# ivclab/CPG

Measured on AMD Instinct MI355X. Metric: images/sec per CPG train-prune-retrain cycle, VGG16 task-1, higher is better.
Workload: dtype f32; 1 GPU; configs[1]: VGG16-BN custom_vgg 224x224, task-1 CPG cycle (finetune -> prune 0.0->0.1 -> recovery, validate after every 20th train step), batch 256 per GPU; task=1, arch=vgg16, global_batch=256, per_gpu_batch=256, parallelism=dp1, epoch_steps=20

## Files before the change

### cpg_amd/_lib.py

```python
import ctypes
import os
import sys

import torch

_HERE = os.path.dirname(os.path.abspath(__file__))
LIB_PATH = os.environ.get('CPG_HIP_LIB') or os.path.join(_HERE, 'lib', 'libcpg_hip.so')

ABI_VERSION = 3
CPG_OK = 0
CPG_E_KRANGE = 2
CPG_E_INVALID = -1
MODE_FINETUNE = 0
MODE_PRUNE = 1



class ConvDesc(ctypes.Structure):
    _fields_ = [(n, ctypes.c_int32) for n in
                ('N', 'C', 'H', 'W', 'K', 'R', 'S', 'stride_h', 'stride_w', 'pad_h', 'pad_w', 'dil_h', 'dil_w', 'groups')]


class PruneResult(ctypes.Structure):
    _fields_ = [('n_candidates', ctypes.c_int64), ('k', ctypes.c_int64), ('n_released', ctypes.c_int64),
# ... 71 lines not shown
    'cpg_bn_workspace_bytes': (_sz, [_i32, _i32, _i32]),
    'cpg_bn_relu_fwd_train': (_int, [_vp, _vp, _vp, _f32, _f32, _vp, _vp, _vp, _vp, _vp, _i32, _i32, _i32, _i32, _vp, _sz, _vp]),
    'cpg_bn_relu_fwd_eval': (_int, [_vp, _vp, _vp, _vp, _vp, _vp, _i32, _i32, _i32, _i32, _vp]),
    'cpg_bn_relu_pool_fwd': (_int, [_vp, _vp, _vp, _f32, _f32, _vp, _vp, _vp, _vp, _vp, _i32, _i32, _i32, _i32, _i32, _vp, _sz, _vp]),
    'cpg_bn_relu_pool_bwd': (_int, [_vp, _vp, _vp, _vp, _vp, _vp, _vp, _vp, _vp, _i32, _i32, _i32, _i32, _i32, _vp, _sz, _vp]),
    'cpg_bn_relu_bwd': (_int, [_vp, _vp, _vp, _vp, _vp, _vp, _vp, _vp, _vp, _i32, _i32, _i32, _i32, _i32, _vp, _sz, _vp]),
    'cpg_conv2d_winograd': (_i32, [_desc, _i32]),
    'cpg_conv2d_bnstats_tiles': (_i32, [_desc]),
    'cpg_conv2d_fwd_bnstats': (_int, [_desc, _vp, _vp, _vp, _f32, _vp, _vp, _vp, _sz, _vp, _sz, _vp]),
    'cpg_conv2d_fwd_bn_eval_supported': (_i32, [_desc]),
    'cpg_conv2d_fwd_bn_eval': (_int, [_desc, _vp, _vp, _vp, _f32, _vp, _vp, _vp, _vp, _vp, _f32, _i32, _vp, _vp, _vp, _sz, _vp]),
    'cpg_conv2d_bf16_supported': (_i32, [_desc]),
    'cpg_conv2d_bf16_workspace_bytes': (_sz, [_desc]),
    'cpg_conv2d_fwd_bf16': (_int, [_desc, _vp, _vp, _vp, _f32, _vp, _vp, _vp, _sz, _vp]),
    'cpg_conv2d_wgrad_bf16_supported': (_i32, [_desc]),
    'cpg_conv2d_wgrad_bf16_workspace_bytes': (_sz, [_desc]),
    'cpg_conv2d_wgrad_bf16': (_int, [_desc, _vp, _vp, _vp, _vp, _f32, _vp, _vp, _vp, _sz, _vp]),
    'cpg_conv2d_fwd_bf16x3': (_int, [_desc, _vp, _vp, _vp, _f32, _vp, _vp, _vp, _sz, _vp]),
    'cpg_conv2d_dgrad_bf16x3': (_int, [_desc, _vp, _vp, _vp, _f32, _vp, _vp, _sz, _vp]),
    'cpg_conv2d_wgrad_bf16x3': (_int, [_desc, _vp, _vp, _vp, _vp, _f32, _vp, _vp, _vp, _sz, _vp]),
    'cpg_conv2d_dgrad_bf16': (_int, [_desc, _vp, _vp, _vp, _f32, _vp, _vp, _sz, _vp]),
    'cpg_conv2d_dgrad_bnbwd_tiles': (_i32, [_desc]),
    'cpg_conv2d_dgrad_bnbwd': (_int, [_desc, _vp, _vp, _vp, _f32, _vp, _vp, _vp, _vp, _vp, _vp, _vp, _sz, _vp, _sz, _vp]),
    'cpg_bn_bwd_from_partials': (_int, [_vp, _i32, _vp, _vp, _vp, _vp, _vp, _vp, _vp, _vp, _vp, _i32, _i32, _i32, _vp, _sz, _vp]),
    'cpg_bn_bwd_finalize_partials': (_int, [_vp, _i32, _i32, _i32, _i32, _vp, _vp, _vp, _vp]),
    'cpg_stem_bn_supported': (_i32, [_desc]),
    'cpg_stem_bn_tiles': (_i32, [_desc]),
    'cpg_stem_bn_stats': (_int, [_desc, _vp, _vp, _vp, _f32, _vp, _vp, _sz, _vp]),
    'cpg_stem_bn_relu_fwd': (_int, [_desc, _vp, _vp, _vp, _f32, _vp, _vp, _vp, _vp, _vp, _vp, _vp]),
    'cpg_stem_bn_relu_bwd_reduce': (_int, [_desc, _vp, _vp, _vp, _f32, _vp, _vp, _vp, _vp, _vp, _vp, _vp, _sz, _vp]),
    'cpg_stem_bn_relu_bwd_apply': (_int, [_desc, _vp, _vp, _vp, _f32, _vp, _vp, _vp, _vp, _vp, _vp, _vp, _vp, _vp]),
    'cpg_stem_bn_wgrad_workspace': (_sz, [_desc]),
    'cpg_stem_bn_relu_bwd_wgrad': (_int, [_desc, _vp, _vp, _vp, _f32, _vp, _vp, _vp, _vp, _vp, _vp, _vp, _vp, _vp, _vp, _sz, _vp]),
    'cpg_bn_stats_finalize_count': (_int, [_vp, _i32, _i32, _i32, _i32, _f32, _f32, _vp, _vp, _vp, _vp, _vp, _vp]),
    'cpg_bn_stats_finalize': (_int, [_vp, _i32, _i32, _i32, _i32, _f32, _f32, _vp, _vp, _vp, _vp, _vp]),
    'cpg_bn_add_relu_mask_bytes': (_sz, [_i32, _i32, _i32]),
    'cpg_bn_add_relu_fwd': (_int, [_vp, _vp, _vp, _vp, _f32, _f32, _vp, _vp, _vp, _vp, _vp, _i32, _i32, _i32, _i32, _vp, _sz, _vp, _vp]),
    'cpg_bn_relu_pool3_supported': (_i32, [_i32, _i32]),
    'cpg_bn_relu_pool3_fwd': (_int, [_vp] * 6 + [_i32] * 4 + [_vp]),
    'cpg_bn_relu_pool3_bwd': (_int, [_vp] * 9 + [_i32] * 5 + [_vp, _sz, _vp]),
    'cpg_bn_add_relu_bwd': (_int, [_vp] * 11 + [_i32] * 4 + [_vp, _sz, _vp, _vp]),
    'cpg_prelu_fwd': (_int, [_vp, _vp, _vp, _vp, _i32, _i32, _i32, _i32, _vp]),
    'cpg_prelu_bwd_bias': (_int, [_vp] * 6 + [_i32] * 4 + [_vp, _sz, _vp]),
    'cpg_prelu_workspace_bytes': (_sz, [_i32, _i32, _i32]),
    'cpg_prelu_bwd': (_int, [_vp, _vp, _vp, _vp, _vp, _i32, _i32, _i32, _i32, _vp, _sz, _vp]),
    'cpg_image_resample_workspace_bytes': (_sz, [ctypes.POINTER(ResampleItem), _i32]),
    'cpg_image_resample': (_int, [_vp, _i64, ctypes.POINTER(ResampleItem), _i32, _vp, _i64, _vp, _sz, _vp]),
    'cpg_image_to_tensor': (_int, [_vp, _i64, ctypes.POINTER(TensorItem), _i32, _i32, _i32, ctypes.POINTER(_f32), ctypes.POINTER(_f32), _vp,
                                           _i64, _vp]),
    'cpg_pair_distance': (_int, [_vp, _i64, _vp, _i64, _i64, _i32, _i32, _vp, _vp, _vp]),
    'cpg_pair_sweep': (_int, [_vp, _vp, _i64, ctypes.POINTER(_f64), _i32, _i32, _vp, _vp, _vp]),
}
EXPORTS = tuple(_SIGNATURES)

_lib = None


class CpgHipError(RuntimeError):
    def __init__(self, fn, code, text):
        super().__init__('%s failed with status %d: %s' % (fn, code, text))
        self.code = code


def lib():
    global _lib
    if _lib is None:
# ... 103 lines not shown
```

### cpg_amd/csrc/conv3x3_stem.hip

```cpp
#include <algorithm>
#include <type_traits>
#include "cpg_dispatch.h"

using namespace cpg;

namespace {

typedef float f32x2 __attribute__((ext_vector_type(2)));
constexpr int ST_R = 8, ST_W = 32;
constexpr int ST_PW = 36;
constexpr int ST_ROWS = ST_R + 2;
constexpr int ST_CMAX = 3, ST_KS = 14;
constexpr int ST_PATCH = ST_CMAX * ST_ROWS * ST_PW;

struct StemGeom {
    int N, C, K, H, W;
    int tiles_x, tiles_y;
    unsigned ntiles;
};

enum { ST_PLAIN = 0, ST_STATS = 1, ST_STATS_ONLY = 2, ST_BN_RELU = 3, ST_BWD_REDUCE = 4, ST_BWD_APPLY = 5, ST_BWD_WGRAD = 6 };
constexpr int ST_TS = 36;
struct StemBn {
    const float *gamma, *beta, *mean, *invstd;
    const float *coef;
    const float *gz;
};

template <int MODE, int NB = 2, bool RAG = false>
__global__ __launch_bounds__(256, 2)
void k_stem_fwd(StemGeom g, const float *__restrict__ x, const float *__restrict__ w, const float *__restrict__ pm, float thr,
                const float *__restrict__ bias, float *__restrict__ y, float *__restrict__ stats, StemBn bn) {
    constexpr bool STATS = MODE == ST_STATS || MODE == ST_STATS_ONLY || MODE == ST_BWD_REDUCE;
    constexpr bool BN = MODE >= ST_BN_RELU;
    constexpr bool STORE = MODE == ST_PLAIN || MODE == ST_STATS || MODE == ST_BN_RELU || MODE == ST_BWD_APPLY;
    constexpr bool WG = MODE == ST_BWD_WGRAD;
    constexpr bool TWO_PASS = STATS || BN;
    __shared__ float smem_all[4 * ST_PATCH];
    __shared__ __attribute__((aligned(16))) float cst[(MODE >= ST_BWD_REDUCE) ? NB * 32 * 8 : 4];
    const int tid = threadIdx.x, lane = tid & 63, wave = __builtin_amdgcn_readfirstlane(tid >> 6);
    if constexpr (MODE >= ST_BWD_REDUCE) {
        if (tid < NB * 32) {
            const bool kv = tid < g.K;
            cst[tid * 8 + 0] = kv ? bn.mean[tid] : 0.0f, cst[tid * 8 + 1] = kv ? bn.invstd[tid] : 0.0f;
            cst[tid * 8 + 2] = kv ? bn.gamma[tid] : 0.0f, cst[tid * 8 + 3] = kv ? bn.beta[tid] : 0.0f;
            cst[tid * 8 + 4] = (MODE >= ST_BWD_APPLY && kv) ? bn.coef[2 * tid] : 0.0f;
            cst[tid * 8 + 5] = (MODE >= ST_BWD_APPLY && kv) ? bn.coef[2 * tid + 1] : 0.0f;
        }
        __syncthreads();
    }
    const int li = lane & 31, lh = lane >> 5;
    float *smem = smem_all + wave * ST_PATCH;
    const int HW = g.H * g.W, CK = g.C * 9;
    __shared__ __attribute__((aligned(16))) float tsm_all[WG ? 4 * 32 * ST_TS : 4];
    float *tsm = tsm_all + (WG ? wave * 32 * ST_TS : 0);
    const int wk = li < CK ? li : 0, wboff = ((wk / 9) * ST_ROWS + (wk % 9) / 3) * ST_PW + wk % 3 + lh;
    f32x16 accw[WG ? NB : 1];
    if constexpr (WG) {
#pragma unroll
        for (int mb = 0; mb < NB; ++mb)
#pragma unroll
            for (int e = 0; e < 16; ++e) accw[mb][e] = 0.0f;
    }

    constexpr bool ALDS = NB == 3 && TWO_PASS;
    __shared__ float a_lds[ALDS ? NB * ST_KS * 64 : 1];
    float A[ALDS ? 1 : NB][ST_KS];
    int boff[ST_KS];
#pragma unroll
    for (int t = 0; t < ST_KS; ++t) {
        const int k = 2 * t + lh;
        const bool kv = k < CK;
#pragma unroll
        for (int mb = 0; mb < NB; ++mb) {
            const int co = mb * 32 + li;
            float v = 0.0f;
            if (kv && co < g.K) {
                v = w[co * CK + k];
                if (pm != nullptr) v *= binarize(pm[co * CK + k], thr);
            }
            if constexpr (ALDS) {
                if (wave == 0) a_lds[(mb * ST_KS + t) * 64 + lane] = v;
            } else {
                A[mb][t] = v;
            }
        }
        const int kk = kv ? k : 0;
        const int c = kk / 9, r = (kk % 9) / 3, s = kk % 3;
        boff[t] = (c * ST_ROWS + r) * ST_PW + s + li;
    }
    constexpr bool HASB = !BN;
    constexpr bool BPASS = HASB && TWO_PASS && NB == 3;
    float bv[HASB ? (BPASS ? 1 : NB) : 1][HASB ? 16 : 1];
    if constexpr (HASB && !BPASS) {
#pragma unroll
        for (int mb = 0; mb < NB; ++mb)
#pragma unroll
            for (int e = 0; e < 16; ++e) {
                const int co = mb * 32 + (e & 3) + 8 * (e >> 2) + 4 * lh;
                bv[mb][e] = (bias != nullptr && co < g.K) ? bias[co] : 0.0f;
            }
    }

    const __amdgpu_buffer_rsrc_t srd_x = __builtin_amdgcn_make_buffer_rsrc((void *)x, 0, g.N * g.C * HW * 4, 0x00020000);
    constexpr int kOOR = (int)0x80000000;
    const int hw_half = lane >> 5, hcol = lane & 31;
    float pc[15], ph;
    auto tile_coords = [&](unsigned tile, int &n, int &y0, int &x0) {
        const unsigned per_img = (unsigned)(g.tiles_x * g.tiles_y);
        n = (int)(tile / per_img);
        const unsigned r = tile % per_img;
        y0 = (int)(r / (unsigned)g.tiles_x) * ST_R, x0 = (int)(r % (unsigned)g.tiles_x) * ST_W;
    };
    auto issue_loads = [&](unsigned tile) {
        int n, y0, x0;
        tile_coords(tile, n, y0, x0);
#pragma unroll
        for (int q = 0; q < 15; ++q) {
            const int item = 2 * q + hw_half, c = item / ST_ROWS, r = item % ST_ROWS;
            const int row = y0 - 1 + r, col = x0 + hcol;
            const bool ok = c < g.C && (unsigned)row < (unsigned)g.H && col < g.W;
            const int off = ok ? (((n * g.C + c) * g.H + row) * g.W + col) * 4 : kOOR;
            pc[q] = __builtin_bit_cast(float, __builtin_amdgcn_raw_buffer_load_b32(srd_x, off, 0, 0));
        }
        {
            const int item = lane >> 1, side = lane & 1, c = item / ST_ROWS, r = item % ST_ROWS;
            const int row = y0 - 1 + r, col = side ? x0 + ST_W : x0 - 1;
            const bool ok = item < ST_CMAX * ST_ROWS && c < g.C && (unsigned)row < (unsigned)g.H && (unsigned)col < (unsigned)g.W;
            const int off = ok ? (((n * g.C + c) * g.H + row) * g.W + col) * 4 : kOOR;
            ph = __builtin_bit_cast(float, __builtin_amdgcn_raw_buffer_load_b32(srd_x, off, 0, 0));
        }
    };
    auto write_patch = [&]() {
#pragma unroll
        for (int q = 0; q < 15; ++q) smem[(2 * q + hw_half) * ST_PW + 1 + hcol] = pc[q];
        if (lane < 2 * ST_CMAX * ST_ROWS) smem[(lane >> 1) * ST_PW + ((lane & 1) ? ST_W + 1 : 0)] = ph;
    };

    if constexpr (ALDS) __syncthreads();
    const unsigned nwaves = gridDim.x * 4, wid = blockIdx.x * 4 + wave;
    if (wid >= g.ntiles) return;
    const int HW4 = HW * 4;
    issue_loads(wid);
    for (unsigned tile = wid; tile < g.ntiles; tile += nwaves) {
        int n, y0, x0;
        tile_coords(tile, n, y0, x0);
        write_patch();
        if (tile + nwaves < g.ntiles) issue_loads(tile + nwaves);
        float s1[16], s2[16];
        auto zero_sums = [&]() {
            if (STATS) {
#pragma unroll
                for (int e = 0; e < 16; ++e) s1[e] = s2[e] = 0.0f;
// ... 67 lines not shown
            for (int mb = MB0; mb < MB1; ++mb)
#pragma unroll
                for (int e = 0; e < 16; ++e) acc[mb][e] = 0.0f;
            const float *prow = smem + j * ST_PW;
#pragma unroll
            for (int t = 0; t < ST_KS; ++t) {
                const float b = prow[boff[t]];
#pragma unroll
                for (int mb = MB0; mb < MB1; ++mb) acc[mb] = __builtin_amdgcn_mfma_f32_32x32x2f32(A[ALDS ? 0 : mb][t], b, acc[mb], 0, 0, 0);
            }
#pragma unroll
            for (int mb = MB0; mb < MB1; ++mb)
#pragma unroll
                for (int e = 0; e < 16; ++e) {
                    const int cu = mb * 32 + (e & 3) + 8 * (e >> 2);
                    const float v = HASB ? acc[mb][e] + bv[(HASB && !BPASS) ? mb : 0][HASB ? e : 0] : acc[mb][e];
                    if constexpr (MODE == ST_PLAIN || MODE == ST_STATS) {
                        __builtin_amdgcn_raw_buffer_store_b32(__builtin_bit_cast(int, v), srd_y, voff_of(mb, e), cu * HW4, 0);
                    }
                    if constexpr (MODE == ST_STATS || MODE == ST_STATS_ONLY) {
                        const float vm = (FULL || pok) ? v : 0.0f;
                        s1[e] += vm;
                        s2[e] = fmaf(vm, vm, s2[e]);
                    }
                    if constexpr (MODE == ST_BN_RELU) {
                        const float z = fmaxf((v - cm[e]) * cis[e] * cga[e] + cbe[e], 0.0f);
                        __builtin_amdgcn_raw_buffer_store_b32(__builtin_bit_cast(int, z), srd_y, voff_of(mb, e), cu * HW4, 0);
                    }
                    if constexpr (MODE >= ST_BWD_REDUCE) {
                        const float *cc = cst + (cu + 4 * lh) * 8 + copq;
                        const f32x4 c4 = *reinterpret_cast<const f32x4 *>(cc);
                        const float xh = (v - c4[0]) * c4[1];
                        const float gm = ((v - c4[0]) * c4[1] * c4[2] + c4[3] > 0.0f) ? gzv[e] : 0.0f;
                        if constexpr (MODE == ST_BWD_REDUCE) {
                            s1[e] += gm;
                            s2[e] = fmaf(gm, xh, s2[e]);
                        } else {
                            const f32x2 c2 = *reinterpret_cast<const f32x2 *>(cc + 4);
                            float gyv = (gm - c2[0] - xh * c2[1]) * (c4[1] * c4[2]);
                            if constexpr (MODE == ST_BWD_APPLY) {
                                __builtin_amdgcn_raw_buffer_store_b32(__builtin_bit_cast(int, gyv), srd_y, voff_of(mb, e), cu * HW4, 0);
                            } else {
                                if (!FULL && !pok) gyv = 0.0f;
                                tsm[((e & 3) + 8 * (e >> 2) + 4 * lh) * ST_TS + (li & 1) * 16 + (li >> 1)] = gyv;
                            }
                        }
                    }
                }
            if constexpr (WG) {
                f32x4 ga[4];
#pragma unroll
                for (int q = 0; q < 4; ++q) ga[q] = *reinterpret_cast<const f32x4 *>(tsm + li * ST_TS + lh * 16 + 4 * q);
                const float *brow = smem + j * ST_PW + wboff;
#pragma unroll
                for (int t = 0; t < 16; ++t)
                    accw[MB0] = __builtin_amdgcn_mfma_f32_32x32x2f32(ga[t >> 2][t & 3], brow[2 * t], accw[MB0], 0, 0, 0);
            }
        };
        auto rows = [&](auto mbsel) {
            if (full) {
#pragma unroll 1
                for (int j = 0; j < ST_R; ++j) row(j, std::true_type{}, mbsel);
            } else {
#pragma unroll 1
                for (int j = 0; j < ST_R; ++j) row(j, std::false_type{}, mbsel);
            }
        };
        auto stats_out = [&](int mb) {
#pragma unroll
            for (int e = 0; e < 16; e += 8) half_wave_sum8(s1 + e), half_wave_sum8(s2 + e);
            if (li == kHalfSumLane) {
#pragma unroll
                for (int e = 0; e < 16; ++e) {
                    const int co = mb * 32 + (e & 3) + 8 * (e >> 2) + 4 * lh;
                    if (RAG && co >= g.K) continue;
                    f32x2 o;
                    o[0] = s1[e], o[1] = s2[e];
                    *reinterpret_cast<f32x2 *>(stats + ((int64_t)co * g.ntiles + tile) * 2) = o;
                }
            }
        };
        if (TWO_PASS) {
            load_bn(0);
            zero_sums();
            rows(std::integral_constant<int, 0>{});
            if (STATS) stats_out(0);
            load_bn(1);
            zero_sums();
            rows(std::integral_constant<int, 1>{});
            if (STATS) stats_out(1);
            if constexpr (NB == 3) {
                load_bn(2);
                zero_sums();
                rows(std::integral_constant<int, 2>{});
                if (STATS) stats_out(2);
            }
        } else {
            rows(std::integral_constant<int, -1>{});
        }
    }
    if constexpr (WG) {
        float *dstw = y + (int64_t)wid * g.K * CK;
#pragma unroll
        for (int mb = 0; mb < NB; ++mb)
#pragma unroll
            for (int e = 0; e < 16; ++e) {
                const int co = mb * 32 + (e & 3) + 8 * (e >> 2) + 4 * lh;
                if (li < CK && co < g.K) dstw[co * CK + li] = accw[mb][e];
            }
    }
}

#define STEM_LAUNCH(MODE, grid, block, shm, stream, ...)                                                          \
    do {                                                                                                          \
        if (g.K == 64) hipLaunchKernelGGL((k_stem_fwd<MODE, 2, false>), grid, block, shm, stream, __VA_ARGS__);   \
        else hipLaunchKernelGGL((k_stem_fwd<MODE, 3, true>), grid, block, shm, stream, __VA_ARGS__);              \
    } while (0)

bool stem_geom(int N, int C, int K, int H, int W, StemGeom &g) {
    if (opt_on(OPT_NO_STEM)) return false;
    if (N < 1 || C < 1 || C > ST_CMAX || K < 64 || K > 96 || H < 1 || W < 1) return false;
    if ((int64_t)N * C * H * W * 4 >= (1ll << 31) || (int64_t)K * H * W * 4 >= (1ll << 31)) return false;
    g.N = N, g.C = C, g.K = K, g.H = H, g.W = W;
    g.tiles_x = (W + ST_W - 1) / ST_W, g.tiles_y = (H + ST_R - 1) / ST_R;
    const int64_t nt = (int64_t)N * g.tiles_x * g.tiles_y;
    if (nt >= (1ll << 31)) return false;
    g.ntiles = (unsigned)nt;
    return true;
}

}

extern "C" int cpg_conv3x3_stem_ok(int N, int C, int K, int H, int W) {
    StemGeom g;
    return stem_geom(N, C, K, H, W, g) ? 1 : 0;
}

extern "C" int cpg_conv3x3_stem_tiles(int N, int C, int K, int H, int W) {
    StemGeom g;
    return stem_geom(N, C, K, H, W, g) ? (int)g.ntiles : 0;
}

// ... 78 lines not shown
    if (!stem_bn_geom(d, g)) return fail(CPG_E_UNSUPPORTED, "cpg_stem_bn_relu_bwd_apply: shape not supported");
    if (bias != nullptr) return fail(CPG_E_UNSUPPORTED, "cpg_stem_bn_relu_bwd_apply: the fused stem takes no conv bias");
    STEM_LAUNCH(ST_BWD_APPLY, dim3(stem_blocks(g)), dim3(256), 0, (hipStream_t)stream_v, g, x, w, pm, thr, bias, gy,
                       (float *)nullptr, StemBn{gamma, beta, mean, invstd, coef, gz});
    CPG_CHECK_LAUNCH("cpg_stem_bn_relu_bwd_apply");
    return CPG_OK;
}

extern "C" size_t cpg_stem_bn_wgrad_workspace(const cpg_conv_desc *d) {
    StemGeom g;
    if (d == nullptr || !stem_bn_geom(d, g)) return 0;
    return (size_t)stem_blocks(g) * 4 * g.K * g.C * 9 * sizeof(float);
}
extern "C" int cpg_stem_bn_relu_bwd_wgrad(const cpg_conv_desc *d, const float *x, const float *w, const float *pm, float thr,
                                          const float *bias, const float *gamma, const float *beta, const float *mean, const float *invstd,
                                          const float *coef, const float *gz, float *gw, float *gpm, void *ws, size_t ws_bytes,
                                          void *stream_v) {
    StemGeom g;
    CPG_REQUIRE(d && x && w && gamma && beta && mean && invstd && coef && gz && gw && ws, "cpg_stem_bn_relu_bwd_wgrad: null pointer");
    CPG_REQUIRE((pm == nullptr) == (gpm == nullptr), "cpg_stem_bn_relu_bwd_wgrad: piggymask and its gradient come as a pair");
    if (!stem_bn_geom(d, g)) return fail(CPG_E_UNSUPPORTED, "cpg_stem_bn_relu_bwd_wgrad: shape not supported");
    if (bias != nullptr) return fail(CPG_E_UNSUPPORTED, "cpg_stem_bn_relu_bwd_wgrad: the fused stem takes no conv bias");
    const unsigned blocks = stem_blocks(g);
    if (ws_bytes < (size_t)blocks * 4 * g.K * g.C * 9 * sizeof(float)) return fail(CPG_E_WORKSPACE, "cpg_stem_bn_relu_bwd_wgrad: workspace too small");
    hipStream_t stream = (hipStream_t)stream_v;
    STEM_LAUNCH(ST_BWD_WGRAD, dim3(blocks), dim3(256), 0, stream, g, x, w, pm, thr, bias, (float *)ws, (float *)nullptr,
                       StemBn{gamma, beta, mean, invstd, coef, gz});
    const int nsplit = (int)std::min<int64_t>((int64_t)g.ntiles, (int64_t)blocks * 4);
    Epilogue ep{gw, nullptr, BIAS_NONE, 1, 1, pm, w, gpm, thr};
    launch_split_reduce((const float *)ws, nsplit, (int64_t)g.K * g.C * 9, 0, ep, stream);
    CPG_CHECK_LAUNCH("cpg_stem_bn_relu_bwd_wgrad");
    return CPG_OK;
}
```

### cpg_amd/csrc/cpg_common.cpp

```cpp
#include "cpg_common.h"
#include <stdarg.h>
#include <stdlib.h>
#include <string.h>
#include <atomic>

namespace cpg {

static thread_local char g_err[512] = "";

char *err_buf() { return g_err; }

int fail(int code, const char *fmt, ...) {
    va_list ap;
    va_start(ap, fmt);
    vsnprintf(g_err, sizeof(g_err), fmt, ap);
    va_end(ap);
    return code;
}

static thread_local PackCtx g_pack = {};
PackCtx &pack_ctx() { return g_pack; }
static thread_local WgradRider g_rider = {};
WgradRider &wgrad_rider() { return g_rider; }

// ... 2 lines not shown
    if (c.mode == PACK_QUERY) {
        c.job = job;
        c.hit = true;
        return 1;
    }
    if (c.mode == PACK_USE && !c.hit) {
        if (c.use == nullptr || c.use_bytes != job.bytes || (((uintptr_t)c.use) & 15) != 0)
            return fail(CPG_E_INVALID, "%s: the packed operand handed in (%zu bytes) is not the one this launch streams (%zu bytes, 16-byte aligned)",
                        what, c.use_bytes, job.bytes);
        *pre = c.use;
        c.hit = true;
        return 2;
    }
    return 0;
}

static std::atomic<int> g_shared_chip{0};
int shared_chip_hint() { return g_shared_chip.load(std::memory_order_relaxed); }

namespace {
enum Kind { BOOL, INT, WINO_KERNEL };
struct OptDef {
    const char *name;
    Kind kind;
};
const OptDef kDefs[OPT_COUNT] = {
    {"CPG_NO_WINO", BOOL},          {"CPG_NO_WINO_WGRAD", BOOL},   {"CPG_NO_WINO_ODD", BOOL},      {"CPG_NO_STEM", BOOL},
    {"CPG_NO_STEM_FUSE", BOOL},     {"CPG_NO_DEAD_SKIP", BOOL},    {"CPG_NO_S2", BOOL},            {"CPG_NO_V14", BOOL},
    {"CPG_DISABLE_CONV3X3", BOOL},  {"CPG_DISABLE_CONV1X1", BOOL}, {"CPG_DISABLE_CONV1X1_WGRAD", BOOL}, {"CPG_DISABLE_PW_GEMM", BOOL},
    {"CPG_C3_FORCE", INT},          {"CPG_C3W_BPC", INT},          {"CPG_W3_PICK", INT},           {"CPG_PWW_BPC", INT},
    {"CPG_STEM_BLOCKS", INT},       {"CPG_WINO_KERNEL", WINO_KERNEL}, {"CPG_WINO_NW", INT},        {"CPG_WINO_PERSIST", INT},
    {"CPG_WINO_GRIDS", INT},        {"CPG_WW_UNITS", INT},         {"CPG_WW_XCD", INT},            {"CPG_PW_TILE", INT},           {"CPG_WG3_SHARE", INT},
    {"CPG_WW_SHARE", INT},          {"CPG_WINO_TAIL", INT},         {"CPG_FC_SMALL", INT},
    {"CPG_NO_WW_RIDER", BOOL},
};

struct Table {
    std::atomic<int> v[OPT_COUNT];
    Table() {
        for (int i = 0; i < OPT_COUNT; ++i) {
            int val = OPT_UNSET;
            if (const char *f = getenv(kDefs[i].name)) {
                switch (kDefs[i].kind) {
                    case BOOL: val = (f[0] == 0 || (f[0] == '0' && f[1] == 0)) ? 0 : 1; break;
                    case INT: val = atoi(f); break;
                    case WINO_KERNEL: val = f[0] == 'b' ? 0 : f[0] == 'p' ? 2 : f[0] == '6' ? 3 : 1; break;
                }
            }
            v[i].store(val, std::memory_order_relaxed);
        }
    }
};
Table g_opts;

int find_opt(const char *name) {
    if (name == nullptr) return -1;
    for (int i = 0; i < OPT_COUNT; ++i)
        if (strcmp(name, kDefs[i].name) == 0) return i;
    return -1;
}
}

int opt(Opt o) { return g_opts.v[o].load(std::memory_order_relaxed); }

}

extern "C" int cpg_set_shared_chip_hint(int32_t shared) {
// ... 19 lines not shown
```

### cpg_amd/csrc/cpg_common.h

```cpp
#pragma once
#include <hip/hip_runtime.h>
#include <stdint.h>
#include <stdio.h>
#include "../../include/cpg_hip.h"

namespace cpg {

char *err_buf();
int fail(int code, const char *fmt, ...);
int shared_chip_hint();

enum Opt {
    OPT_NO_WINO,
    OPT_NO_WINO_WGRAD,
    OPT_NO_WINO_ODD,
    OPT_NO_STEM,
    OPT_NO_STEM_FUSE,
    OPT_NO_DEAD_SKIP,
    OPT_NO_S2,
    OPT_NO_V14,
    OPT_DISABLE_CONV3X3,
    OPT_DISABLE_CONV1X1,
    OPT_DISABLE_CONV1X1_WGRAD,
    OPT_DISABLE_PW_GEMM,
    OPT_C3_FORCE,
    OPT_C3W_BPC,
    OPT_W3_PICK,
    OPT_PWW_BPC,
    OPT_STEM_BLOCKS,
    OPT_WINO_KERNEL,
    OPT_WINO_NW,
    OPT_WINO_PERSIST,
    OPT_WINO_GRIDS,
    OPT_WW_UNITS,
    OPT_WW_XCD,
    OPT_PW_TILE,
    OPT_WG3_SHARE,
    OPT_WW_SHARE,
    OPT_WINO_TAIL,
    OPT_FC_SMALL,
    OPT_NO_WW_RIDER,
    OPT_COUNT
};
constexpr int OPT_UNSET = INT32_MIN;
int opt(Opt o);
inline bool opt_on(Opt o) { const int v = opt(o); return v != OPT_UNSET && v != 0; }
inline int opt_or(Opt o, int dflt) { const int v = opt(o); return v == OPT_UNSET ? dflt : v; }

struct PackJob {
    int family;
    int K, C;
    int a, b, c, d;
    long long total;
    size_t bytes;
};
enum { PACK_NONE = 0, PACK_QUERY = 1, PACK_USE = 2 };
struct PackCtx {
    int mode;
    bool hit;
    PackJob job;
    const float *use;
    size_t use_bytes;
};
PackCtx &pack_ctx();
inline bool pack_query() { return pack_ctx().mode == PACK_QUERY; }
int pack_site(const PackJob &job, const float **pre, const char *what);
int pack_jobs_launch(const PackJob *ja, float *dst_a, const PackJob *jb, float *dst_b, const float *w, const float *pm, float thr,
                     hipStream_t stream);

struct WgradRider {
    bool armed;
    const float *y, *gz, *table;
    float *gy;
    int N, C, HW;
// ... 47 lines not shown
```

### cpg_amd/models/fused_bn.py

```python
import ctypes

import torch
import torch.nn as nn

from .. import _lib
from .layers import BiasGradSink, BnBwdHint, _conv_desc

ENABLED = True
ENABLE_BWD_HINT = False
ENABLE_WGRAD_RIDER = True
RELU_BYTE_MASK = True
FUSE_STEM = True
FUSE_STEM_WGRAD = True
FUSE_SKIP_ADD = True


def _batch_stats(stats, nbt, N, C, HW, eps, momentum, running_mean, running_var, training, device):
    if not training:
        return running_mean, torch.rsqrt(running_var + eps), nbt
    mean = torch.empty(C, dtype=torch.float32, device=device)
    invstd = torch.empty(C, dtype=torch.float32, device=device)
    if stats is not None:
        args = (_lib.dptr(stats, name='bn partial sums'), stats.shape[1], N, C, HW, float(eps), float(momentum),
                _lib.dptr(running_mean, name='running_mean'), _lib.dptr(running_var, name='running_var'), _lib.dptr(mean), _lib.dptr(invstd))
# ... 338 lines not shown
    @staticmethod
    def forward(ctx, x, weight, pm, thr, gamma, beta, running_mean, running_var, eps, momentum, nbt=None):
        x = x.contiguous()
        w = weight.contiguous()
        p = None if pm is None else pm.contiguous()
        d = _conv_desc(x.shape, w.shape, (1, 1), (1, 1), (1, 1), 1)
        s = _lib.stream_ptr()
        thr = float(thr)
        N, K, H, W = x.shape[0], w.shape[0], x.shape[2], x.shape[3]
        tiles = _lib.lib().cpg_stem_bn_tiles(ctypes.byref(d))
        stats = torch.empty((K, tiles, 2), dtype=torch.float32, device=x.device)
        _lib.call('cpg_stem_bn_stats', ctypes.byref(d), _lib.dptr(x, name='input'), _lib.dptr(w, name='weight'), _lib.dptr(p, name='piggymask'),
                  thr, None, _lib.dptr(stats), stats.numel() * 4, s)
        mean, invstd, nbt = _batch_stats(stats, nbt, N, K, H * W, eps, momentum, running_mean, running_var, True, x.device)
        z = torch.empty((N, K, H, W), dtype=torch.float32, device=x.device)
        _lib.call('cpg_stem_bn_relu_fwd', ctypes.byref(d), _lib.dptr(x), _lib.dptr(w), _lib.dptr(p), thr, None, _lib.dptr(gamma, name='bn.weight'),
                  _lib.dptr(beta, name='bn.bias'), _lib.dptr(mean), _lib.dptr(invstd), _lib.dptr(z), s)
        _count(nbt)
        ctx.save_for_backward(x, w, p, gamma, beta, mean, invstd)
        ctx.desc, ctx.thr, ctx.tiles = d, thr, tiles
        return z

    @staticmethod
    def backward(ctx, gz):
        x, w, p, gamma, beta, mean, invstd = ctx.saved_tensors
        d, thr, tiles = ctx.desc, ctx.thr, ctx.tiles
        gz = gz.contiguous()
        L = _lib.lib()
        s = _lib.stream_ptr()
        N, K, H, W = x.shape[0], w.shape[0], x.shape[2], x.shape[3]
        partials = torch.empty((K, tiles, 2), dtype=torch.float32, device=x.device)
        args = (ctypes.byref(d), _lib.dptr(x), _lib.dptr(w), _lib.dptr(p), thr, None, _lib.dptr(gamma), _lib.dptr(beta), _lib.dptr(mean),
                _lib.dptr(invstd))
        _lib.call('cpg_stem_bn_relu_bwd_reduce', *args, _lib.dptr(gz, name='grad_output'), _lib.dptr(partials), partials.numel() * 4, s)
        dgamma, dbeta = torch.empty_like(gamma), torch.empty_like(beta)
        coef = torch.empty(2 * K, dtype=torch.float32, device=x.device)
        _lib.call('cpg_bn_bwd_finalize_partials', _lib.dptr(partials), tiles, N, K, H * W, _lib.dptr(dgamma), _lib.dptr(dbeta), _lib.dptr(coef), s)
        gw = gpm = None
        if ctx.needs_input_grad[1] or (p is not None and ctx.needs_input_grad[2]):
            gw = torch.empty_like(w)
            gpm = None if p is None else torch.empty_like(p)
            if FUSE_STEM_WGRAD:
                ws, nbytes = _lib.workspace(L.cpg_stem_bn_wgrad_workspace(ctypes.byref(d)), x.device)
                _lib.call('cpg_stem_bn_relu_bwd_wgrad', *args, _lib.dptr(coef), _lib.dptr(gz), _lib.dptr(gw), _lib.dptr(gpm), _lib.dptr(ws),
                          nbytes, s)
            else:
                gy = torch.empty((N, K, H, W), dtype=torch.float32, device=x.device)
                _lib.call('cpg_stem_bn_relu_bwd_apply', *args, _lib.dptr(coef), _lib.dptr(gz), _lib.dptr(gy), s)
                ws, nbytes = _lib.workspace(L.cpg_conv2d_workspace_bytes(ctypes.byref(d)), x.device)
                _lib.call('cpg_conv2d_wgrad', ctypes.byref(d), _lib.dptr(x), _lib.dptr(gy), _lib.dptr(w), _lib.dptr(p), thr, _lib.dptr(gw),
                          _lib.dptr(gpm), None, _lib.dptr(ws), nbytes, s)
        return (None, gw, gpm, None, dgamma, dbeta) + (None,) * 5


def stem_conv_bn_relu(conv, bn, x):
    if not (ENABLED and FUSE_STEM and FusedSequential.fuse and hasattr(conv, 'forward_with_bn_stats')
            and _stats_from_conv(bn, FusedSequential.fuse_stats, x, need_grad=True)
            and x.dim() == 4 and x.dtype == torch.float32 and not x.requires_grad
            and conv.bias is None and conv._math() == 'fp32' and tuple(conv.kernel_size) == (3, 3) and tuple(conv.stride) == (1, 1)
            and tuple(conv.padding) == (1, 1) and tuple(conv.dilation) == (1, 1) and conv.groups == 1 and x.shape[0] > 0
            and x.shape[1] == conv.weight.shape[1] and bn.weight.dtype == torch.float32):
        return None
    d = _conv_desc(x.shape, conv.weight.shape, (1, 1), (1, 1), (1, 1), 1)
    if not _lib.lib().cpg_stem_bn_supported(ctypes.byref(d)):
        return None
    return _StemConvBnReluFn.apply(x, conv.weight, conv.piggymask, conv.info['threshold'], bn.weight, bn.bias, bn.running_mean, bn.running_var,
                                   bn.eps, bn.momentum, bn.num_batches_tracked)


def conv_bn_act_skip(conv, bn, act, x):
    if (ENABLED and FUSE_SKIP_ADD and hasattr(conv, 'forward_with_skip') and x.is_cuda and torch.is_grad_enabled() and x.requires_grad
            and conv._math() == 'fp32' and conv.kernel_size == (1, 1) and conv.stride == (1, 1) and conv.in_channels % 16 == 0
            and conv.out_channels % 16 == 0):
        y, stats, skip = conv.forward_with_skip(x)
        if (stats is not None and _stats_from_conv(bn, FusedSequential.fuse_stats) and (act is None or type(act) is nn.ReLU)
# ... 83 lines not shown
```

### include/cpg_hip.h

```cpp
#ifndef CPG_HIP_H
#define CPG_HIP_H

#include <stddef.h>
#include <stdint.h>

#ifdef __cplusplus
extern "C" {
#endif

#define CPG_ABI_VERSION 3

#define CPG_OK 0
#define CPG_E_INVALID (-1)
#define CPG_E_UNSUPPORTED (-2)
#define CPG_E_WORKSPACE (-3)
#define CPG_E_KRANGE 2
#define CPG_E_HIP_BASE 1000

#define CPG_MODE_FINETUNE 0
#define CPG_MODE_PRUNE 1

typedef struct cpg_conv_desc {
    int32_t N, C, H, W;
    int32_t K;
// ... 145 lines not shown
                        const float *bias, float *y, void *workspace, size_t workspace_bytes, void *stream);
int cpg_conv2d_dgrad_bf16(const cpg_conv_desc *desc, const float *gy, const float *w, const float *piggymask, float threshold,
                          float *gx, void *workspace, size_t workspace_bytes, void *stream);

int32_t cpg_conv2d_dgrad_bnbwd_tiles(const cpg_conv_desc *desc);
int cpg_conv2d_dgrad_bnbwd(const cpg_conv_desc *desc, const float *gy, const float *w, const float *piggymask, float threshold,
                           const float *ypre, const float *gamma, const float *beta, const float *mean, const float *invstd,
                           float *gm, float *partials, size_t partial_bytes, void *workspace, size_t workspace_bytes, void *stream);
int cpg_bn_bwd_from_partials(const float *partials, int32_t tiles, const float *x, const float *gm, const float *gamma,
                             const float *beta, const float *mean, const float *invstd, float *gx, float *dgamma, float *dbeta,
                             int32_t N, int32_t C, int32_t HW, void *workspace, size_t workspace_bytes, void *stream);

int cpg_bn_bwd_finalize_partials(const float *partials, int32_t tiles, int32_t N, int32_t C, int32_t HW, float *dgamma, float *dbeta,
                                 float *coef, void *stream);

int32_t cpg_stem_bn_supported(const cpg_conv_desc *desc);
int32_t cpg_stem_bn_tiles(const cpg_conv_desc *desc);
int cpg_stem_bn_stats(const cpg_conv_desc *desc, const float *x, const float *w, const float *piggymask, float threshold,
                      const float *bias, float *stats, size_t stats_bytes, void *stream);
int cpg_stem_bn_relu_fwd(const cpg_conv_desc *desc, const float *x, const float *w, const float *piggymask, float threshold,
                         const float *bias, const float *gamma, const float *beta, const float *mean, const float *invstd, float *z,
                         void *stream);
int cpg_stem_bn_relu_bwd_reduce(const cpg_conv_desc *desc, const float *x, const float *w, const float *piggymask, float threshold,
                                const float *bias, const float *gamma, const float *beta, const float *mean, const float *invstd,
                                const float *gz, float *partials, size_t partials_bytes, void *stream);
int cpg_stem_bn_relu_bwd_apply(const cpg_conv_desc *desc, const float *x, const float *w, const float *piggymask, float threshold,
                               const float *bias, const float *gamma, const float *beta, const float *mean, const float *invstd,
                               const float *coef, const float *gz, float *gy, void *stream);
size_t cpg_stem_bn_wgrad_workspace(const cpg_conv_desc *desc);
int cpg_stem_bn_relu_bwd_wgrad(const cpg_conv_desc *desc, const float *x, const float *w, const float *piggymask, float threshold,
                               const float *bias, const float *gamma, const float *beta, const float *mean, const float *invstd,
                               const float *coef, const float *gz, float *gw, float *gpm, void *workspace, size_t workspace_bytes,
                               void *stream);

size_t cpg_bn_add_relu_mask_bytes(int32_t N, int32_t C, int32_t HW);
int cpg_bn_add_relu_fwd(const float *x, const float *res, const float *gamma, const float *beta, float eps,
                        float momentum, float *running_mean, float *running_var, float *mean, float *invstd, float *y,
                        int32_t N, int32_t C, int32_t HW, int32_t train, void *ws, size_t ws_bytes, void *stream, uint8_t *relu_mask);
int cpg_bn_add_relu_bwd(const float *x, const float *out, const float *gy, const float *gamma, const float *beta,
                        const float *mean, const float *invstd, float *gx, float *gz, float *dgamma, float *dbeta, int32_t N,
                        int32_t C, int32_t HW, int32_t train, void *ws, size_t ws_bytes, void *stream, const uint8_t *relu_mask);

int cpg_bn_relu_pool_fwd(const float *x, const float *gamma, const float *beta, float eps, float momentum,
                         float *running_mean, float *running_var, float *mean, float *invstd, float *y_pooled,
                         int32_t N, int32_t C, int32_t H, int32_t W, int32_t train, void *ws, size_t ws_bytes,
                         void *stream);
int cpg_bn_relu_pool_bwd(const float *x, const float *g_pooled, const float *gamma, const float *beta,
                         const float *mean, const float *invstd, float *gx, float *dgamma, float *dbeta,
                         int32_t N, int32_t C, int32_t H, int32_t W, int32_t train, void *ws, size_t ws_bytes,
                         void *stream);

int32_t cpg_bn_relu_pool3_supported(int32_t H, int32_t W);
int cpg_bn_relu_pool3_fwd(const float *x, const float *gamma, const float *beta, const float *mean, const float *invstd,
                          float *y_pooled, int32_t N, int32_t C, int32_t H, int32_t W, void *stream);
int cpg_bn_relu_pool3_bwd(const float *x, const float *g_pooled, const float *gamma, const float *beta, const float *mean,
                          const float *invstd, float *gx, float *dgamma, float *dbeta, int32_t N, int32_t C, int32_t H,
                          int32_t W, int32_t train, void *workspace, size_t workspace_bytes, void *stream);

size_t cpg_prelu_workspace_bytes(int32_t N, int32_t C, int32_t HW);
int cpg_prelu_bwd(const float *x, const float *gy, const float *slope, float *gx, float *gslope, int32_t N,
                  int32_t C, int32_t HW, int32_t n_slopes, void *ws, size_t ws_bytes, void *stream);
int cpg_prelu_bwd_bias(const float *x, const float *gy, const float *slope, float *gx, float *gslope, float *gbias, int32_t N,
                       int32_t C, int32_t HW, int32_t n_slopes, void *workspace, size_t workspace_bytes, void *stream);
int cpg_prelu_fwd(const float *x, const float *residual, const float *slope, float *y, int32_t N, int32_t C, int32_t HW,
                  int32_t n_slopes, void *stream);

// ... 31 lines not shown
```

Before: 2403 images/sec.

## Fold stem BN-backward weight gradient into single pass using gram-matrix sums

Replaces the two-pass stem backward (reduce pass, then a second full pass recomputing conv output to form the weight gradient) with one pass. That pass accumulates the BN partials, raw gm·x weight sums, and a 28x28 input gram matrix (with a ones row) via MFMA. A small merge kernel sums the per-wave partials in double precision, and a combine kernel rebuilds the exact BN-corrected weight gradient algebraically from those sums, so the second read of the input and gz is avoided. In exchange it uses a larger workspace, adds two small kernels, and relies on double-precision algebra that could change rounding.

```diff
diff --git a/cpg_amd/_lib.py b/cpg_amd/_lib.py
--- a/cpg_amd/_lib.py
+++ b/cpg_amd/_lib.py
@@ -127,6 +127,10 @@
     'cpg_stem_bn_relu_bwd_apply': (_int, [_desc, _vp, _vp, _vp, _f32, _vp, _vp, _vp, _vp, _vp, _vp, _vp, _vp, _vp]),
     'cpg_stem_bn_wgrad_workspace': (_sz, [_desc]),
     'cpg_stem_bn_relu_bwd_wgrad': (_int, [_desc, _vp, _vp, _vp, _f32, _vp, _vp, _vp, _vp, _vp, _vp, _vp, _vp, _vp, _vp, _sz, _vp]),
+    'cpg_stem_bn_sums_workspace': (_sz, [_desc]),
+    'cpg_stem_bn_sums_launches': (_i64, []),
+    'cpg_stem_bn_relu_bwd_sums': (_int, [_desc, _vp, _vp, _vp, _f32, _vp, _vp, _vp, _vp, _vp, _vp, _vp, _sz, _vp, _sz, _vp]),
+    'cpg_stem_bn_bwd_combine': (_int, [_desc, _vp, _vp, _f32, _vp, _vp, _vp, _vp, _vp, _sz, _vp, _vp, _vp]),
     'cpg_bn_stats_finalize_count': (_int, [_vp, _i32, _i32, _i32, _i32, _f32, _f32, _vp, _vp, _vp, _vp, _vp, _vp]),
     'cpg_bn_stats_finalize': (_int, [_vp, _i32, _i32, _i32, _i32, _f32, _f32, _vp, _vp, _vp, _vp, _vp]),
     'cpg_bn_add_relu_mask_bytes': (_sz, [_i32, _i32, _i32]),
diff --git a/cpg_amd/csrc/conv3x3_stem.hip b/cpg_amd/csrc/conv3x3_stem.hip
--- a/cpg_amd/csrc/conv3x3_stem.hip
+++ b/cpg_amd/csrc/conv3x3_stem.hip
@@ -1,4 +1,5 @@
 #include <algorithm>
+#include <atomic>
 #include <type_traits>
 #include "cpg_dispatch.h"
 
@@ -19,7 +20,8 @@
     unsigned ntiles;
 };
 
-enum { ST_PLAIN = 0, ST_STATS = 1, ST_STATS_ONLY = 2, ST_BN_RELU = 3, ST_BWD_REDUCE = 4, ST_BWD_APPLY = 5, ST_BWD_WGRAD = 6 };
+enum { ST_PLAIN = 0, ST_STATS = 1, ST_STATS_ONLY = 2, ST_BN_RELU = 3, ST_BWD_REDUCE = 4, ST_BWD_APPLY = 5, ST_BWD_WGRAD = 6, ST_BWD_SUMS = 7 };
+constexpr int ST_QN = 32;
 constexpr int ST_TS = 36;
 struct StemBn {
     const float *gamma, *beta, *mean, *invstd;
@@ -31,10 +33,12 @@
 __global__ __launch_bounds__(256, 2)
 void k_stem_fwd(StemGeom g, const float *__restrict__ x, const float *__restrict__ w, const float *__restrict__ pm, float thr,
                 const float *__restrict__ bias, float *__restrict__ y, float *__restrict__ stats, StemBn bn) {
-    constexpr bool STATS = MODE == ST_STATS || MODE == ST_STATS_ONLY || MODE == ST_BWD_REDUCE;
+    constexpr bool SUMS = MODE == ST_BWD_SUMS;
+    constexpr bool STATS = MODE == ST_STATS || MODE == ST_STATS_ONLY || MODE == ST_BWD_REDUCE || SUMS;
     constexpr bool BN = MODE >= ST_BN_RELU;
     constexpr bool STORE = MODE == ST_PLAIN || MODE == ST_STATS || MODE == ST_BN_RELU || MODE == ST_BWD_APPLY;
-    constexpr bool WG = MODE == ST_BWD_WGRAD;
+    constexpr bool WG = MODE == ST_BWD_WGRAD || SUMS;
+    constexpr bool COEF = MODE == ST_BWD_APPLY || MODE == ST_BWD_WGRAD;
     constexpr bool TWO_PASS = STATS || BN;
     __shared__ float smem_all[4 * ST_PATCH];
     __shared__ __attribute__((aligned(16))) float cst[(MODE >= ST_BWD_REDUCE) ? NB * 32 * 8 : 4];
@@ -44,8 +48,8 @@
             const bool kv = tid < g.K;
             cst[tid * 8 + 0] = kv ? bn.mean[tid] : 0.0f, cst[tid * 8 + 1] = kv ? bn.invstd[tid] : 0.0f;
             cst[tid * 8 + 2] = kv ? bn.gamma[tid] : 0.0f, cst[tid * 8 + 3] = kv ? bn.beta[tid] : 0.0f;
-            cst[tid * 8 + 4] = (MODE >= ST_BWD_APPLY && kv) ? bn.coef[2 * tid] : 0.0f;
-            cst[tid * 8 + 5] = (MODE >= ST_BWD_APPLY && kv) ? bn.coef[2 * tid + 1] : 0.0f;
+            cst[tid * 8 + 4] = (COEF && kv) ? bn.coef[2 * tid] : 0.0f;
+            cst[tid * 8 + 5] = (COEF && kv) ? bn.coef[2 * tid + 1] : 0.0f;
         }
         __syncthreads();
     }
@@ -56,6 +60,11 @@
     float *tsm = tsm_all + (WG ? wave * 32 * ST_TS : 0);
     const int wk = li < CK ? li : 0, wboff = ((wk / 9) * ST_ROWS + (wk % 9) / 3) * ST_PW + wk % 3 + lh;
     f32x16 accw[WG ? NB : 1];
+    f32x16 accq;
+    if constexpr (SUMS) {
+#pragma unroll
+        for (int e = 0; e < 16; ++e) accq[e] = 0.0f;
+    }
     if constexpr (WG) {
 #pragma unroll
         for (int mb = 0; mb < NB; ++mb)
@@ -63,7 +72,7 @@
             for (int e = 0; e < 16; ++e) accw[mb][e] = 0.0f;
     }
 
-    constexpr bool ALDS = NB == 3 && TWO_PASS;
+    constexpr bool ALDS = (NB == 3 && TWO_PASS) || SUMS;
     __shared__ float a_lds[ALDS ? NB * ST_KS * 64 : 1];
     float A[ALDS ? 1 : NB][ST_KS];
     int boff[ST_KS];
@@ -115,10 +124,12 @@
     auto issue_loads = [&](unsigned tile) {
         int n, y0, x0;
         tile_coords(tile, n, y0, x0);
+        int hq = hw_half, cq = hcol;
+        if constexpr (SUMS) asm volatile("" : "+v"(hq), "+v"(cq));
 #pragma unroll
         for (int q = 0; q < 15; ++q) {
-            const int item = 2 * q + hw_half, c = item / ST_ROWS, r = item % ST_ROWS;
-            const int row = y0 - 1 + r, col = x0 + hcol;
+            const int item = 2 * q + hq, c = item / ST_ROWS, r = item % ST_ROWS;
+            const int row = y0 - 1 + r, col = x0 + cq;
             const bool ok = c < g.C && (unsigned)row < (unsigned)g.H && col < g.W;
             const int off = ok ? (((n * g.C + c) * g.H + row) * g.W + col) * 4 : kOOR;
             pc[q] = __builtin_bit_cast(float, __builtin_amdgcn_raw_buffer_load_b32(srd_x, off, 0, 0));
@@ -252,10 +263,13 @@
                         const f32x4 c4 = *reinterpret_cast<const f32x4 *>(cc);
                         const float xh = (v - c4[0]) * c4[1];
                         const float gm = ((v - c4[0]) * c4[1] * c4[2] + c4[3] > 0.0f) ? gzv[e] : 0.0f;
-                        if constexpr (MODE == ST_BWD_REDUCE) {
+                        if constexpr (MODE == ST_BWD_REDUCE || SUMS) {
                             s1[e] += gm;
                             s2[e] = fmaf(gm, xh, s2[e]);
-                        } else {
+                        }
+                        if constexpr (SUMS) {
+                            tsm[((e & 3) + 8 * (e >> 2) + 4 * lh) * ST_TS + (li & 1) * 16 + (li >> 1)] = gm;
+                        } else if constexpr (MODE != ST_BWD_REDUCE) {
                             const f32x2 c2 = *reinterpret_cast<const f32x2 *>(cc + 4);
                             float gyv = (gm - c2[0] - xh * c2[1]) * (c4[1] * c4[2]);
                             if constexpr (MODE == ST_BWD_APPLY) {
@@ -275,6 +289,15 @@
 #pragma unroll
                 for (int t = 0; t < 16; ++t)
                     accw[MB0] = __builtin_amdgcn_mfma_f32_32x32x2f32(ga[t >> 2][t & 3], brow[2 * t], accw[MB0], 0, 0, 0);
+                if constexpr (SUMS && MB0 == 0) {
+#pragma unroll
+                    for (int t = 0; t < 16; ++t) {
+                        const float b = brow[2 * t];
+                        float qa = li == 27 ? 1.0f : b;
+                        if (!FULL && !(x0 + 2 * t + lh < g.W && y0 + j < g.H)) qa = 0.0f;
+                        accq = __builtin_amdgcn_mfma_f32_32x32x2f32(qa, b, accq, 0, 0, 0);
+                    }
+                }
             }
         };
         auto rows = [&](auto mbsel) {
@@ -289,6 +312,11 @@
         auto stats_out = [&](int mb) {
 #pragma unroll
             for (int e = 0; e < 16; e += 8) half_wave_sum8(s1 + e), half_wave_sum8(s2 + e);
+            unsigned ntl = 0;
+            if constexpr (SUMS) {
+                ntl = g.ntiles;
+                asm volatile("" : "+s"(ntl));
+            }
             if (li == kHalfSumLane) {
 #pragma unroll
                 for (int e = 0; e < 16; ++e) {
@@ -296,7 +324,8 @@
                     if (RAG && co >= g.K) continue;
                     f32x2 o;
                     o[0] = s1[e], o[1] = s2[e];
-                    *reinterpret_cast<f32x2 *>(stats + ((int64_t)co * g.ntiles + tile) * 2) = o;
+                    if constexpr (SUMS) *reinterpret_cast<f32x2 *>(stats + ((int64_t)co * ntl + tile) * 2) = o;
+                    else *reinterpret_cast<f32x2 *>(stats + ((int64_t)co * g.ntiles + tile) * 2) = o;
                 }
             }
         };
@@ -321,13 +350,20 @@
     }
     if constexpr (WG) {
         float *dstw = y + (int64_t)wid * g.K * CK;
+        int lq = li, hq = lh;
+        if constexpr (SUMS) asm volatile("" : "+v"(lq), "+v"(hq));
 #pragma unroll
         for (int mb = 0; mb < NB; ++mb)
 #pragma unroll
             for (int e = 0; e < 16; ++e) {
-                const int co = mb * 32 + (e & 3) + 8 * (e >> 2) + 4 * lh;
-                if (li < CK && co < g.K) dstw[co * CK + li] = accw[mb][e];
-            }
+                const int co = mb * 32 + (e & 3) + 8 * (e >> 2) + 4 * hq;
+                if (lq < CK && co < g.K) dstw[co * CK + lq] = accw[mb][e];
+            }
+        if constexpr (SUMS) {
+            float *dstq = y + (int64_t)nwaves * g.K * CK + (int64_t)wid * (ST_QN * ST_QN);
+#pragma unroll
+            for (int e = 0; e < 16; ++e) dstq[((e & 3) + 8 * (e >> 2) + 4 * hq) * ST_QN + lq] = accq[e];
+        }
     }
 }
 
@@ -472,3 +508,102 @@
     CPG_CHECK_LAUNCH("cpg_stem_bn_relu_bwd_wgrad");
     return CPG_OK;
 }
+
+namespace {
+constexpr int ST_MCH = 32;
+std::atomic<int64_t> g_sums_launches{0};
+
+bool stem_sums_geom(const cpg_conv_desc *d, StemGeom &g) {
+    if (opt_on(OPT_STEM_BWD_TWO_PASS)) return false;
+    return stem_bn_geom(d, g) && g.K == 64;
+}
+size_t stem_sums_bytes(const StemGeom &g) {
+    const size_t nw = (size_t)stem_blocks(g) * 4, na = (size_t)g.K * g.C * 9, tot = na + ST_QN * ST_QN;
+    return nw * tot * sizeof(float) + (size_t)ST_MCH * tot * sizeof(double);
+}
+
+__global__ __launch_bounds__(256) void k_stem_sums_merge(const float *__restrict__ pa, const float *__restrict__ pq, int nsplit, int na,
+                                                         double *__restrict__ mid) {
+    const int tot = na + ST_QN * ST_QN, idx = blockIdx.x * 256 + threadIdx.x;
+    if (idx >= tot * ST_MCH) return;
+    const int e = idx % tot, c = idx / tot, per = (nsplit + ST_MCH - 1) / ST_MCH;
+    const int k0 = c * per, k1 = k0 + per < nsplit ? k0 + per : nsplit;
+    const float *p = e < na ? pa + e : pq + (e - na);
+    const int64_t stride = e < na ? na : ST_QN * ST_QN;
+    double s = 0.0;
+    for (int k = k0; k < k1; ++k) s += (double)p[k * stride];
+    mid[idx] = s;
+}
+
+__global__ __launch_bounds__(256) void k_stem_sums_combine(const double *__restrict__ mid, int K, int CK, const float *__restrict__ w,
+                                                           const float *__restrict__ pm, float thr, const float *__restrict__ gamma,
+                                                           const float *__restrict__ mean, const float *__restrict__ invstd,
+                                                           const float *__restrict__ coef, Epilogue ep) {
+    __shared__ double qs[ST_QN * ST_QN];
+    const int na = K * CK, tot = na + ST_QN * ST_QN;
+    for (int i = threadIdx.x; i < ST_QN * ST_QN; i += 256) {
+        double s = 0.0;
+        for (int c = 0; c < ST_MCH; ++c) s += mid[(int64_t)c * tot + na + i];
+        qs[i] = s;
+    }
+    __syncthreads();
+    const int e = blockIdx.x * 256 + threadIdx.x;
+    if (e >= na) return;
+    const int k = e / CK, t = e % CK;
+    double a = 0.0;
+    for (int c = 0; c < ST_MCH; ++c) a += mid[(int64_t)c * tot + e];
+    double wq = 0.0;
+    for (int u = 0; u < CK; ++u) {
+        float wv = w[k * CK + u];
+        if (pm != nullptr) wv *= binarize(pm[k * CK + u], thr);
+        wq += (double)wv * qs[u * ST_QN + t];
+    }
+    const double P = qs[27 * ST_QN + t], is = invstd[k], m1 = coef[2 * k], m2 = coef[2 * k + 1];
+    const double gv = is * (double)gamma[k] * (a - m1 * P - m2 * is * (wq - (double)mean[k] * P));
+    epilogue_store(ep, e, (float)gv);
+}
+}
+
+extern "C" size_t cpg_stem_bn_sums_workspace(const cpg_conv_desc *d) {
+    StemGeom g;
+    if (d == nullptr || !stem_sums_geom(d, g)) return 0;
+    return stem_sums_bytes(g);
+}
+extern "C" int64_t cpg_stem_bn_sums_launches(void) { return g_sums_launches.load(std::memory_order_relaxed); }
+
+extern "C" int cpg_stem_bn_relu_bwd_sums(const cpg_conv_desc *d, const float *x, const float *w, const float *pm, float thr,
+                                         const float *bias, const float *gamma, const float *beta, const float *mean, const float *invstd,
+                                         const float *gz, float *partials, size_t partials_bytes, void *ws, size_t ws_bytes, void *stream_v) {
+    StemGeom g;
+    CPG_REQUIRE(d && x && w && gamma && beta && mean && invstd && gz && partials && ws, "cpg_stem_bn_relu_bwd_sums: null pointer");
+    if (!stem_sums_geom(d, g)) return fail(CPG_E_UNSUPPORTED, "cpg_stem_bn_relu_bwd_sums: shape not supported");
+    if (bias != nullptr) return fail(CPG_E_UNSUPPORTED, "cpg_stem_bn_relu_bwd_sums: the fused stem takes no conv bias");
+    if (partials_bytes < (size_t)g.K * g.ntiles * 2 * sizeof(float)) return fail(CPG_E_WORKSPACE, "cpg_stem_bn_relu_bwd_sums: partial-sum buffer too small");
+    if (ws_bytes < stem_sums_bytes(g)) return fail(CPG_E_WORKSPACE, "cpg_stem_bn_relu_bwd_sums: workspace too small");
+    hipLaunchKernelGGL((k_stem_fwd<ST_BWD_SUMS, 2, false>), dim3(stem_blocks(g)), dim3(256), 0, (hipStream_t)stream_v, g, x, w, pm, thr, bias,
+                       (float *)ws, partials, StemBn{gamma, beta, mean, invstd, nullptr, gz});
+    CPG_CHECK_LAUNCH("cpg_stem_bn_relu_bwd_sums");
+    g_sums_launches.fetch_add(1, std::memory_order_relaxed);
+    return CPG_OK;
+}
+
+extern "C" int cpg_stem_bn_bwd_combine(const cpg_conv_desc *d, const float *w, const float *pm, float thr, const float *gamma,
+                                       const float *mean, const float *invstd, const float *coef, void *ws, size_t ws_bytes, float *gw,
+                                       float *gpm, void *stream_v) {
+    StemGeom g;
+    CPG_REQUIRE(d && w && gamma && mean && invstd && coef && ws && gw, "cpg_stem_bn_bwd_combine: null pointer");
+    CPG_REQUIRE((pm == nullptr) == (gpm == nullptr), "cpg_stem_bn_bwd_combine: piggymask and its gradient come as a pair");
+    if (!stem_sums_geom(d, g)) return fail(CPG_E_UNSUPPORTED, "cpg_stem_bn_bwd_combine: shape not supported");
+    if (ws_bytes < stem_sums_bytes(g)) return fail(CPG_E_WORKSPACE, "cpg_stem_bn_bwd_combine: workspace too small");
+    hipStream_t stream = (hipStream_t)stream_v;
+    const int nw = (int)stem_blocks(g) * 4, na = g.K * g.C * 9, tot = na + ST_QN * ST_QN;
+    const int nsplit = (int)std::min<int64_t>((int64_t)g.ntiles, nw);
+    const float *pa = (const float *)ws, *pq = pa + (size_t)nw * na;
+    double *mid = (double *)(pa + (size_t)nw * tot);
+    hipLaunchKernelGGL(k_stem_sums_merge, dim3((unsigned)((tot * ST_MCH + 255) / 256)), dim3(256), 0, stream, pa, pq, nsplit, na, mid);
+    Epilogue ep{gw, nullptr, BIAS_NONE, 1, 1, pm, w, gpm, thr};
+    hipLaunchKernelGGL(k_stem_sums_combine, dim3((unsigned)((na + 255) / 256)), dim3(256), 0, stream, (const double *)mid, g.K, g.C * 9, w, pm,
+                       thr, gamma, mean, invstd, coef, ep);
+    CPG_CHECK_LAUNCH("cpg_stem_bn_bwd_combine");
+    return CPG_OK;
+}
diff --git a/cpg_amd/csrc/cpg_common.cpp b/cpg_amd/csrc/cpg_common.cpp
--- a/cpg_amd/csrc/cpg_common.cpp
+++ b/cpg_amd/csrc/cpg_common.cpp
@@ -58,7 +58,7 @@
     {"CPG_STEM_BLOCKS", INT},       {"CPG_WINO_KERNEL", WINO_KERNEL}, {"CPG_WINO_NW", INT},        {"CPG_WINO_PERSIST", INT},
     {"CPG_WINO_GRIDS", INT},        {"CPG_WW_UNITS", INT},         {"CPG_WW_XCD", INT},            {"CPG_PW_TILE", INT},           {"CPG_WG3_SHARE", INT},
     {"CPG_WW_SHARE", INT},          {"CPG_WINO_TAIL", INT},         {"CPG_FC_SMALL", INT},
-    {"CPG_NO_WW_RIDER", BOOL},
+    {"CPG_NO_WW_RIDER", BOOL},      {"CPG_STEM_BWD_TWO_PASS", BOOL},
 };
 
 struct Table {
diff --git a/cpg_amd/csrc/cpg_common.h b/cpg_amd/csrc/cpg_common.h
--- a/cpg_amd/csrc/cpg_common.h
+++ b/cpg_amd/csrc/cpg_common.h
@@ -40,6 +40,7 @@
     OPT_WINO_TAIL,
     OPT_FC_SMALL,
     OPT_NO_WW_RIDER,
+    OPT_STEM_BWD_TWO_PASS,
     OPT_COUNT
 };
 constexpr int OPT_UNSET = INT32_MIN;
diff --git a/cpg_amd/models/fused_bn.py b/cpg_amd/models/fused_bn.py
--- a/cpg_amd/models/fused_bn.py
+++ b/cpg_amd/models/fused_bn.py
@@ -394,15 +394,25 @@
         partials = torch.empty((K, tiles, 2), dtype=torch.float32, device=x.device)
         args = (ctypes.byref(d), _lib.dptr(x), _lib.dptr(w), _lib.dptr(p), thr, None, _lib.dptr(gamma), _lib.dptr(beta), _lib.dptr(mean),
                 _lib.dptr(invstd))
-        _lib.call('cpg_stem_bn_relu_bwd_reduce', *args, _lib.dptr(gz, name='grad_output'), _lib.dptr(partials), partials.numel() * 4, s)
+        want_gw = ctx.needs_input_grad[1] or (p is not None and ctx.needs_input_grad[2])
+        sums_bytes = L.cpg_stem_bn_sums_workspace(ctypes.byref(d)) if (want_gw and FUSE_STEM_WGRAD) else 0
+        if sums_bytes:
+            ws, nbytes = _lib.workspace(sums_bytes, x.device)
+            _lib.call('cpg_stem_bn_relu_bwd_sums', *args, _lib.dptr(gz, name='grad_output'), _lib.dptr(partials), partials.numel() * 4,
+                      _lib.dptr(ws), nbytes, s)
+        else:
+            _lib.call('cpg_stem_bn_relu_bwd_reduce', *args, _lib.dptr(gz, name='grad_output'), _lib.dptr(partials), partials.numel() * 4, s)
         dgamma, dbeta = torch.empty_like(gamma), torch.empty_like(beta)
         coef = torch.empty(2 * K, dtype=torch.float32, device=x.device)
         _lib.call('cpg_bn_bwd_finalize_partials', _lib.dptr(partials), tiles, N, K, H * W, _lib.dptr(dgamma), _lib.dptr(dbeta), _lib.dptr(coef), s)
         gw = gpm = None
-        if ctx.needs_input_grad[1] or (p is not None and ctx.needs_input_grad[2]):
+        if want_gw:
             gw = torch.empty_like(w)
             gpm = None if p is None else torch.empty_like(p)
-            if FUSE_STEM_WGRAD:
+            if sums_bytes:
+                _lib.call('cpg_stem_bn_bwd_combine', ctypes.byref(d), _lib.dptr(w), _lib.dptr(p), thr, _lib.dptr(gamma), _lib.dptr(mean),
+                          _lib.dptr(invstd), _lib.dptr(coef), _lib.dptr(ws), nbytes, _lib.dptr(gw), _lib.dptr(gpm), s)
+            elif FUSE_STEM_WGRAD:
                 ws, nbytes = _lib.workspace(L.cpg_stem_bn_wgrad_workspace(ctypes.byref(d)), x.device)
                 _lib.call('cpg_stem_bn_relu_bwd_wgrad', *args, _lib.dptr(coef), _lib.dptr(gz), _lib.dptr(gw), _lib.dptr(gpm), _lib.dptr(ws),
                           nbytes, s)
diff --git a/include/cpg_hip.h b/include/cpg_hip.h
--- a/include/cpg_hip.h
+++ b/include/cpg_hip.h
@@ -201,6 +201,15 @@
                                const float *bias, const float *gamma, const float *beta, const float *mean, const float *invstd,
                                const float *coef, const float *gz, float *gw, float *gpm, void *workspace, size_t workspace_bytes,
                                void *stream);
+size_t cpg_stem_bn_sums_workspace(const cpg_conv_desc *desc);
+int64_t cpg_stem_bn_sums_launches(void);
+int cpg_stem_bn_relu_bwd_sums(const cpg_conv_desc *desc, const float *x, const float *w, const float *piggymask, float threshold,
+                              const float *bias, const float *gamma, const float *beta, const float *mean, const float *invstd,
+                              const float *gz, float *partials, size_t partials_bytes, void *workspace, size_t workspace_bytes,
+                              void *stream);
+int cpg_stem_bn_bwd_combine(const cpg_conv_desc *desc, const float *w, const float *piggymask, float threshold, const float *gamma,
+                            const float *mean, const float *invstd, const float *coef, void *workspace, size_t workspace_bytes,
+                            float *gw, float *gpm, void *stream);
 
 size_t cpg_bn_add_relu_mask_bytes(int32_t N, int32_t C, int32_t HW);
 int cpg_bn_add_relu_fwd(const float *x, const float *res, const float *gamma, const float *beta, float eps,
```

Result: no change. 2416 images/sec (median of 6 runs) (+0.5%).
